# SvenGronauer/distributedTensorFlow

Measured on AMD Instinct MI355X. Metric: images/sec (whole node) ResNet-50 synthetic ImageNet at 1/2/4/8 MI355X, higher is better.
Workload: dtype bf16; 1 GPU; model=resnet50, global_batch=1984, per_gpu_batch=1984, image_size=224, parallelism=dp1, impl=dtf, optimizer=momentum0.9+wd1e-4, lr 0.1*B/256 warmup500+cosine, backend=auto, native_ext=distributedtensorflow_amd/_lib/_dtf_hip.cpython-310-x86_64-linux-gnu.so

## Files before the change

csrc/kernels/batchnorm.hip:

```cpp
#include <stdexcept>

#include "launch.h"

namespace {

constexpr int kThreads = 256;

static int g_bn_stats_blocks = 1024;

inline int stats_grid(long M, int C, int* rows_per_block) {
  const int tpr = C / 8;
  const int rpi = kThreads / tpr;
  long target_blocks = g_bn_stats_blocks;
  long rpb = (M + target_blocks - 1) / target_blocks;
  rpb = ((rpb + rpi - 1) / rpi) * rpi;
  if (rpb < rpi) rpb = rpi;
  *rows_per_block = (int)rpb;
  return (int)((M + rpb - 1) / rpb);
}

constexpr int kUnroll = 4;

DTF_DEV void relu_mask8(float* g, const float* xv, uint32_t mbyte, uint4 yraw, int kind,
                        const float* ksc, const float* ksh) {
  if (kind == 1) {
#pragma unroll
    for (int i = 0; i < 8; ++i) g[i] = (mbyte >> i) & 1u ? g[i] : 0.f;
  } else if (kind == 2) {
#pragma unroll
    for (int i = 0; i < 8; ++i) g[i] = __builtin_fmaf(xv[i], ksc[i], ksh[i]) > 0.f ? g[i] : 0.f;
  } else if (kind == 3) {
    float yv[8];
    unpack8(yraw, yv);
#pragma unroll
    for (int i = 0; i < 8; ++i) g[i] = yv[i] > 0.f ? g[i] : 0.f;
  }
}

DTF_DEV void load8cg(const float* __restrict__ p, int cg, float* v) {
  const float4 a = reinterpret_cast<const float4*>(p)[cg * 2];
  const float4 b = reinterpret_cast<const float4*>(p)[cg * 2 + 1];
  v[0] = a.x; v[1] = a.y; v[2] = a.z; v[3] = a.w; v[4] = b.x; v[5] = b.y; v[6] = b.z; v[7] = b.w;
}

typedef uint32_t u32x4_nt __attribute__((ext_vector_type(4)));
// ... 617 lines not shown
```

csrc/kernels/bindings.cpp:

```cpp
#include <hip/hip_runtime.h>
#include <pybind11/pybind11.h>
#include <pybind11/stl.h>

#include <algorithm>
#include <stdexcept>
#include <string>
#include <vector>

#include "launch.h"

namespace py = pybind11;

namespace dlp {
struct Device { int32_t device_type; int32_t device_id; };
struct DataType { uint8_t code; uint8_t bits; uint16_t lanes; };
struct Tensor { void* data; Device device; int32_t ndim; DataType dtype; int64_t* shape;
                int64_t* strides; uint64_t byte_offset; };
struct Managed { Tensor t; void* ctx; void (*deleter)(Managed*); };
constexpr int32_t kROCM = 10;
struct Ctx { int64_t shape[1]; int64_t strides[1]; uintptr_t ptr; int device; bool opened; };
void deleter(Managed* m) {
  auto* c = static_cast<Ctx*>(m->ctx);
  if (c->opened) dtf_ipc_close(c->ptr, c->device);
  else dtf_ipc_free(c->ptr, c->device);
// ... 446 lines not shown
             eeta, eps, gscale, nesterov, P<float>(partial), P<int>(nonfinite), S(st));
    check_launch("lars");
  });
  m.def("sumsq", [](uintptr_t x, long n, uintptr_t out, uintptr_t st) {
    dtf_sumsq(P<const float>(x), n, P<float>(out), S(st));
    check_launch("sumsq");
  });
  m.def("cast_f32_bf16", [](uintptr_t x, uintptr_t y, long n, uintptr_t st) {
    dtf_cast_f32_bf16(P<const float>(x), P<bf16_t>(y), n, S(st));
    check_launch("cast_f32_bf16");
  });
  m.def("conv_igemm", [](uintptr_t x, uintptr_t w, uintptr_t y, std::vector<int> geom,
                         std::vector<int> dh, std::vector<int> dw, int bk, uintptr_t st,
                         uintptr_t stats, std::vector<uintptr_t> bnb, uintptr_t acc_src,
                         uintptr_t acc_mask, uintptr_t bias, int relu, uintptr_t bnl_sc,
                         uintptr_t bnl_sh, uintptr_t bnl_y) {
    ConvGeom g = conv_geom("conv_igemm", geom);
    g.acc_src = P<const bf16_t>(acc_src);
    g.acc_mask = P<const uint8_t>(acc_mask);
    g.bias = P<const float>(bias);
    g.relu = relu;
    if (g.acc == 2 && (!g.acc_src || !g.acc_mask))
      throw std::runtime_error("conv_igemm: acc 2 needs acc_src and acc_mask");
    g.lsc = P<const float>(bnl_sc);
    g.lsh = P<const float>(bnl_sh);
    g.ly = P<bf16_t>(bnl_y);
    const BnBwdEpi e = bnb_epi("conv_igemm", bnb, 9);
    dtf_conv_igemm(P<const bf16_t>(x), P<const bf16_t>(w), P<bf16_t>(y), g,
                   make_taps<TapTable>(dh, dw), bk, P<float>(stats), e, S(st));
    check_launch("conv_igemm");
  }, py::arg("x"), py::arg("w"), py::arg("y"), py::arg("geom"), py::arg("dh"), py::arg("dw"),
     py::arg("bk"), py::arg("stream"), py::arg("stats") = 0,
     py::arg("bnb") = std::vector<uintptr_t>{}, py::arg("acc_src") = 0, py::arg("acc_mask") = 0,
     py::arg("bias") = 0, py::arg("relu") = 0, py::arg("bnl_sc") = 0, py::arg("bnl_sh") = 0,
     py::arg("bnl_y") = 0);
  m.def("conv_igemm_grouped", [](uintptr_t x, uintptr_t y, std::vector<int> geom,
                                 std::vector<uintptr_t> wts, std::vector<int> oh0,
                                 std::vector<int> ow0, std::vector<int> kpad,
                                 std::vector<std::vector<int>> dh, std::vector<std::vector<int>> dw,
                                 uintptr_t st, std::vector<uintptr_t> bnb, std::vector<int> row0) {
    if (geom.size() != 17) throw std::runtime_error("conv_igemm_grouped: geom needs 17 ints");
    const size_t n = wts.size();
    if (oh0.size() != n || ow0.size() != n || kpad.size() != n || dh.size() != n ||
        dw.size() != n || (!bnb.empty() && row0.size() != n))
      throw std::runtime_error("conv_igemm_grouped: per-class lists differ in length");
    const ConvGeom g = conv_geom("conv_igemm_grouped", geom);
    const BnBwdEpi e = bnb_epi("conv_igemm_grouped", bnb, 8);
    std::vector<const bf16_t*> w(n);
    for (size_t i = 0; i < n; ++i) w[i] = P<const bf16_t>(wts[i]);
    const bool ok = dtf_conv_igemm_grouped(P<const bf16_t>(x), P<bf16_t>(y), g, (int)n, w.data(),
                                           oh0.data(), ow0.data(), kpad.data(), dh, dw, e,
                                           row0.empty() ? nullptr : row0.data(), S(st));
    if (ok) check_launch("conv_igemm_grouped");
    return ok;
  });
  m.def("gemm_conv_part_images", &dtf_gemm_conv_part_images);
  m.def("gemm_set_pp2_strided", &dtf_gemm_set_pp2_strided);
  m.def("conv_bnl_ok", [](std::vector<int> geom, std::vector<int> dh, std::vector<int> dw) {
    const ConvGeom g = conv_geom("conv_bnl_ok", geom);
    return dtf_conv_bnl_ok(g, make_taps<TapTable>(dh, dw));
  });
  m.def("bn_bwd_finalize_g", [](uintptr_t part, int G, long M, int C, uintptr_t gamma,
                                uintptr_t mean, uintptr_t invstd, uintptr_t dg, uintptr_t db,
                                uintptr_t a, uintptr_t b, uintptr_t c, int accumulate,
                                uintptr_t st) {
    dtf_bn_bwd_finalize_g(P<const float>(part), G, M, C, P<const float>(gamma),
                          P<const float>(mean), P<const float>(invstd), P<float>(dg), P<float>(db),
                          P<float>(a), P<float>(b), P<float>(c), accumulate, S(st));
    check_launch("bn_bwd_finalize_g");
  });
  m.def("conv_wgrad", [](uintptr_t x, uintptr_t dy, uintptr_t dw_out, uintptr_t ws,
                         std::vector<int> geom, std::vector<int> dh, std::vector<int> dw,
                         int splits, uintptr_t st, int tr_mode, int accumulate) {
    if (geom.size() != 10) throw std::runtime_error("conv_wgrad: geom needs 10 ints");
    WgradGeom g{geom[0], geom[1], geom[2], geom[3], geom[4], geom[5], geom[6], geom[7], geom[8],
// ... 235 lines not shown
```

csrc/kernels/common.h:

```cpp
#pragma once
#include <hip/hip_runtime.h>
#include <stdint.h>

#define DTF_DEV __device__ __forceinline__

typedef uint16_t bf16_t;
typedef __attribute__((ext_vector_type(8))) short bf16x8_t;
typedef __attribute__((ext_vector_type(4))) short bf16x4_t;
typedef __attribute__((ext_vector_type(4))) float f32x4_t;
typedef __attribute__((ext_vector_type(16))) float f32x16_t;

DTF_DEV float bf2f(bf16_t v) { return __builtin_bit_cast(float, ((uint32_t)v) << 16); }
DTF_DEV bf16_t f2bf(float f) { return __builtin_bit_cast(bf16_t, (__bf16)f); }

DTF_DEV void unpack8(const uint4& v, float* f) {
  const uint32_t w[4] = {v.x, v.y, v.z, v.w};
#pragma unroll
  for (int i = 0; i < 4; ++i) {
    f[2 * i] = __builtin_bit_cast(float, w[i] << 16);
    f[2 * i + 1] = __builtin_bit_cast(float, w[i] & 0xffff0000u);
  }
}
DTF_DEV uint32_t pack2(float a, float b) {
  return (uint32_t)f2bf(a) | ((uint32_t)f2bf(b) << 16);
// ... 65 lines not shown
#define DTF_WAIT_VM(n) asm volatile("s_waitcnt vmcnt(" #n ")" ::: "memory")
template <int N>
DTF_DEV void wait_vm() {
  static_assert(N >= 0 && N < 64, "vmcnt range");
  asm volatile("s_waitcnt vmcnt(%0)" ::"n"(N) : "memory");
}
DTF_DEV void raw_barrier() {
  asm volatile("" ::: "memory");
  __builtin_amdgcn_s_barrier();
  asm volatile("" ::: "memory");
}

DTF_DEV float bn_bwd_dx(float a, float dz, float b, float x, float c) {
  return __builtin_fmaf(a, dz, b * x) + c;
}

DTF_DEV void pool3s2_gather(const uint4 (&dyr)[4], const uint2 (&amr)[4], int a, int b, int P,
                            int Q, float (&g)[4][8]) {
#pragma unroll
  for (int k = 0; k < 4; ++k)
#pragma unroll
    for (int e = 0; e < 8; ++e) g[k][e] = 0.f;
#pragma unroll
  for (int da = 0; da < 2; ++da) {
    if (a + da >= P) continue;
#pragma unroll
    for (int db = 0; db < 2; ++db) {
      if (b + db >= Q) continue;
      float gv[8];
      unpack8(dyr[da * 2 + db], gv);
// ... 49 lines not shown
```

csrc/kernels/conv.hip:

```cpp
#include <algorithm>
#include <stdexcept>
#include <string>
#include <vector>

#include "launch.h"

DTF_DEV uint4 acc_add8(const ConvGeom& g, const bf16_t* Y, long off, uint4 v) {
  float a[8], b[8];
  unpack8(v, a);
  if (g.acc == 2) {
    unpack8(*reinterpret_cast<const uint4*>(g.acc_src + off), b);
    const uint32_t m = g.acc_mask[off >> 3];
#pragma unroll
    for (int e = 0; e < 8; ++e) b[e] = (m >> e) & 1u ? b[e] : 0.f;
  } else {
    unpack8(*reinterpret_cast<const uint4*>(Y + off), b);
  }
#pragma unroll
  for (int e = 0; e < 8; ++e) a[e] += b[e];
  return pack8(a);
}

static int g_small_k = 31;

// ... 666 lines not shown
  static constexpr int LDC = NT + 8;
  static constexpr size_t LDS = (size_t)(PIXAL * C + 2 * WST) * 2;
  static constexpr size_t lds(int st, int nstg = 2) {
    return (size_t)(st * PIXAL * C + nstg * WST) * 2;
  }
  static constexpr size_t LDS_FREG = (size_t)PIXAL * C * 2;
  static_assert(M % (16 * WMW) == 0 && NT % (16 * WNW) == 0, "halo tiling");
  static_assert((size_t)M * LDC * 2 + (size_t)2 * NT * (kThreads / NT) * 4 <= (size_t)PIXAL * C * 2,
                "halo epilogue must fit in the patch region");
};

template <int C>
DTF_DEV int halo_swz(int u) { return C == 64 ? (((u >> 1) & 3) << 1) : ((u & 7) << 1); }

template <int C, int W, int WMW, int NT, int ST = 1, bool FREG = false, bool BNB = false,
          int NSTG = 2, bool BNL = false, int BNLP = 0>
__global__ void __launch_bounds__(kThreads * ST, ST == 1 ? 2 : 1)
conv3x3_halo_kernel(const bf16_t* __restrict__ X, const bf16_t* __restrict__ Wt,
                    bf16_t* __restrict__ Y, const ConvGeom g, const TapTable taps,
                    float* __restrict__ stats, const BnBwdEpi bnb) {
  using H = HaloCfg<C, W, WMW, NT>;
  static_assert(!BNL || (!FREG && ST == 1 && !BNB), "BN on load: the forward ring kernel");
  extern __shared__ __attribute__((aligned(16))) bf16_t lds[];
  const int tid = threadIdx.x & (kThreads - 1), lane = tid & 63;
  const int wall = __builtin_amdgcn_readfirstlane((int)threadIdx.x >> 6);
  const int sid = wall >> 2, wave = wall & 3;
  bf16_t* const patch = lds + sid * (H::PIXAL * C);
  bf16_t* const wst = lds + ST * (H::PIXAL * C);
  float* const bnl_prm = reinterpret_cast<float*>(wst + NSTG * H::WST);
  if constexpr (BNL) {
    for (int t = tid; t < C / 4; t += kThreads) {
      const int ch = t >> 1, half = t & 1;
      reinterpret_cast<float4*>(bnl_prm)[ch * 4 + half] =
          *reinterpret_cast<const float4*>(g.lsc + 4 * t);
      reinterpret_cast<float4*>(bnl_prm)[ch * 4 + 2 + half] =
          *reinterpret_cast<const float4*>(g.lsh + 4 * t);
    }
  }
  const int wm = wave / H::WNW, wn = wave % H::WNW;
  const int tiles_h = g.H / kHaloTH;
  const int tm = blockIdx.x * ST + sid;
  const bool live = tm < g.N * tiles_h;
  const int n = live ? tm / tiles_h : 0, h0 = live ? (tm % tiles_h) * kHaloTH : 0;
  const int n0 = blockIdx.y * NT;
  const i32x4_t rx = rsrc_quad(X + (long)n * g.H * g.W * g.C, (uint32_t)g.H * g.W * g.C * 2u);
  const i32x4_t rw = rsrc_quad(Wt, (uint32_t)g.Kout * g.Kpad * 2u);
  const uint32_t lds_patch = lds_addr(patch), lds_w = lds_addr(wst);

  {
    constexpr int CPP = H::ROWB / 16;
    const int lp = lane / CPP, slot = lane % CPP;
    for (int q = wave; q < H::PIXAL / H::PPI; q += 4) {
      const int pix = q * H::PPI + lp;
// ... 3 lines not shown
      const bool ok = live && pix < H::PIX && (unsigned)h < (unsigned)g.H &&
                      (unsigned)w < (unsigned)g.W;
      const uint32_t off = ok ? (uint32_t)(((h * g.W + w) * C + chunk * 8) * 2) : kOOB;
      dma16(rx, lds_patch + (uint32_t)q * 1024u, off);
    }
  }
  constexpr int OCPR = NT / 8;
  constexpr int OROWS = kThreads / OCPR;
  constexpr int NR = H::M / OROWS;
  static_assert(H::M % OROWS == 0, "halo epilogue rows");
  const long ybase = ((long)n * g.H + h0) * g.W;
  const int oc = tid % OCPR;
  const bool col_ok = n0 + oc * 8 < g.Kout;
  uint4 xpre[BNB ? NR : 1];
  uint32_t mpre[BNB ? NR : 1];
  if constexpr (BNB) {
#pragma unroll
    for (int k = 0; k < NR; ++k) {
      const long off = (ybase + tid / OCPR + k * OROWS) * g.Kout + n0 + oc * 8;
      const bool ok = live && col_ok;
      xpre[k] = ok ? *reinterpret_cast<const uint4*>(bnb.x + off) : make_uint4(0, 0, 0, 0);
      mpre[k] = (ok && bnb.mkind == 1) ? (uint32_t)bnb.mask[off >> 3] : 0u;
    }
  }
  const int lp8 = lane >> 3, slot8 = lane & 7;
  auto issue_w = [&](int step, int stage) {
    const int t = step / H::KS, s = step - t * H::KS;
#pragma unroll
    for (int i = 0; i < NT / (32 * ST); ++i) {
      const int q = wall + 4 * ST * i;
      const int row = q * 8 + lp8;
      const int chunk = slot8 ^ ((row >> 1) & 7);
      const int kr = n0 + row;
      const uint32_t off = (t < taps.n && kr < g.Kout)
                               ? (uint32_t)((kr * g.Kpad + t * C + s * 64 + chunk * 8) * 2) : kOOB;
      dma16(rw, lds_w + (uint32_t)(stage * H::WST) * 2u + (uint32_t)q * 1024u, off);
    }
// ... 64 lines not shown
        for (int i = 0; i < H::MF; ++i) {
          const int p = pbase[i] + dpix;
          const bf16x8_t af = *reinterpret_cast<const bf16x8_t*>(
              patch + p * C + ((pch ^ halo_swz<C>(ubase[i] + dupix)) << 3));
#pragma unroll
          for (int j = 0; j < H::NF; ++j)
            acc[i][j] = __builtin_amdgcn_mfma_f32_16x16x32_bf16(af, cur[ks][j], acc[i][j], 0, 0, 0);
        }
      }
      __builtin_amdgcn_sched_barrier(0);
      if (step + D < NSTEP) ldB(step + D, cur);
      __builtin_amdgcn_sched_barrier(0);
    }
  } else {
  const int nsteps = taps.n * H::KS;
  for (int step = 0; step < nsteps; ++step) {
    if constexpr (kYoung == 0) DTF_WAIT_VM(0);
    else if constexpr (kYoung == 1) DTF_WAIT_VM(1);
    else if constexpr (kYoung == 2) DTF_WAIT_VM(2);
    else if constexpr (kYoung == 3) DTF_WAIT_VM(3);
    else if constexpr (kYoung == 4) DTF_WAIT_VM(4);
    else if constexpr (kYoung == 6) DTF_WAIT_VM(6);
    else DTF_WAIT_VM(8);
    __syncthreads();
    if constexpr (BNL) {
      if (step == 0) {
        constexpr int CPP = H::ROWB / 16;
        constexpr int ITEMS = (H::PIX * CPP + kThreads - 1) / kThreads;
#pragma unroll
        for (int k = 0; k < ITEMS; ++k) {
          const int idx = tid + k * kThreads;
          const int pix = idx / CPP, slot = idx - pix * CPP;
          const int pr = pix / H::PW, pc = pix - pr * H::PW;
          const int h = h0 - 1 + pr, w = pc - 1;
          if (idx >= H::PIX * CPP || (unsigned)h >= (unsigned)g.H || (unsigned)w >= (unsigned)g.W)
            continue;
          const int lch = slot ^ halo_swz<C>(pr * W + pc);
          uint4* pp = reinterpret_cast<uint4*>(patch + pix * C + slot * 8);
// ... 307 lines not shown
                            : conv3x3_halo_kernel<C, W, WMW, NT, 1, false, false, 2, true>;
#else
    auto kern = conv3x3_halo_kernel<C, W, WMW, NT, 1, false, false, 2, true>;
#endif
    const size_t lds = Hc::lds(1) + (size_t)2 * C * sizeof(float);
    static bool attr[2] = {false, false};
    if (!attr[g_bnl_probe ? 1 : 0]) {
      HIP_CHECK(hipFuncSetAttribute((const void*)kern, hipFuncAttributeMaxDynamicSharedMemorySize,
                                    (int)lds));
      attr[g_bnl_probe ? 1 : 0] = true;
    }
    hipLaunchKernelGGL(kern, dim3((unsigned)tiles, g.Kout / NT), dim3(kThreads), lds, st,
                       X, Wt, Y, g, taps, stats, bnb);
    return;
  }
  if (!freg_on && (nstg == 3 || nstg == 4)) {
    if (bnb.part) {
      constexpr size_t scratch =
          (size_t)Hc::M * Hc::LDC * 2 + (size_t)(kThreads / (NT / 8)) * 2 * NT * 4;
      const size_t base = Hc::lds(1, nstg);
      const size_t lds = base > scratch ? base : scratch;
      if (nstg == 3) launch_halo_ring<C, W, WMW, NT, 1, true, 3>(X, Wt, Y, g, taps, stats, bnb, tiles, lds, st);
      else launch_halo_ring<C, W, WMW, NT, 1, true, 4>(X, Wt, Y, g, taps, stats, bnb, tiles, lds, st);
    } else if (strips == 2) {
      if (nstg == 3) launch_halo_ring<C, W, WMW, NT, 2, false, 3>(X, Wt, Y, g, taps, stats, bnb, tiles, Hc::lds(2, 3), st);
      else launch_halo_ring<C, W, WMW, NT, 2, false, 4>(X, Wt, Y, g, taps, stats, bnb, tiles, Hc::lds(2, 4), st);
    } else {
      if (nstg == 3) launch_halo_ring<C, W, WMW, NT, 1, false, 3>(X, Wt, Y, g, taps, stats, bnb, tiles, Hc::lds(1, 3), st);
      else launch_halo_ring<C, W, WMW, NT, 1, false, 4>(X, Wt, Y, g, taps, stats, bnb, tiles, Hc::lds(1, 4), st);
    }
// ... 79 lines not shown
  if (use_conv_gemm(g, taps)) return (int)(((long)g.N * g.P * g.Q + 255) / 256);
  if (g.C % 32 == 0 && use_halo(g, taps)) return g.N * (g.H / kHaloTH);
  if (use_stem_halo(g, taps)) return g.N * (g.P / kStemTH);
  const long M = (long)g.N * g.P * g.Q;
  return dtf_conv_stats_rows(M, g.Kout, g.C, taps.n, 0);
}

static int g_conv_nt = 0;
void dtf_conv_set_nt(int v) { g_conv_nt = v; }

bool dtf_conv_bnl_ok(const ConvGeom& g, const TapTable& taps) {
  const int fam = halo_family(g, taps);
  if (!fam || (g_halo_freg & fam) || (g_halo_st & fam)) return false;
  const int nstg = (g_halo_stages >> (fam == 1 ? 0 : 4)) & 15;
  return nstg != 3 && nstg != 4;
}

void dtf_conv_igemm(const bf16_t* X, const bf16_t* Wt, bf16_t* Y, const ConvGeom& g_in,
                    const TapTable& taps, int bk, float* stats, const BnBwdEpi& bnb,
                    hipStream_t st) {
  ConvGeom g = g_in;
  g.nt = g_conv_nt;
  if (bnb.part && (stats || !bnb.x || !bnb.mean || !bnb.invstd ||
                   (bnb.mkind == 1 && !bnb.mask) || (bnb.mkind == 2 && !(bnb.fsc && bnb.fsh))))
    throw std::runtime_error("conv: bad fused BN-backward epilogue arguments");
  if (taps.n <= 0 || taps.n > DTF_MAX_TAPS) throw std::runtime_error("conv: bad tap count");
  if (g.Kout % 8) throw std::runtime_error("conv: Kout % 8 != 0");
  const double ibytes = 2.0 * g.H * g.W * g.C, wbytes = 2.0 * g.Kout * g.Kpad;
  const double m = (double)g.N * g.P * g.Q;
  const double span = (double)(255 / (g.P * g.Q) + 2);
// ... 2 lines not shown
    throw std::runtime_error("conv: image / filter too large for 32-bit buffer offsets");
  const bool narrow = g.Kout <= 64;
  const bool epi = g.bias || g.relu;
  if (epi && (bnb.part || g.acc))
    throw std::runtime_error("conv: fused bias/ReLU epilogue excludes BN / accumulate epilogues");
  if (g.ly) {
    if (!dtf_conv_bnl_ok(g, taps) || !g.lsc || !g.lsh || bnb.part || epi)
      throw std::runtime_error("conv: BN on load needs a halo-family forward conv");
    const int tiles = g.N * (g.H / kHaloTH);
    if (halo_family(g, taps) == 1)
      launch_halo<64, 56, 2, 64>(X, Wt, Y, g, taps, stats, bnb, tiles, 1, st);
    else
      launch_halo<128, 28, 1, 128>(X, Wt, Y, g, taps, stats, bnb, tiles, 1, st);
    return;
  }
  if (!bnb.part && use_stem_halo(g, taps)) {
    using Sc = StemCfg<112>;
    static bool attr = false;
    if (!attr) {
      HIP_CHECK(hipFuncSetAttribute((const void*)conv_stem_halo_kernel<112>,
                                    hipFuncAttributeMaxDynamicSharedMemorySize, (int)Sc::LDS));
      attr = true;
    }
    hipLaunchKernelGGL(conv_stem_halo_kernel<112>, dim3((unsigned)(g.N * (g.P / kStemTH))),
                       dim3(kThreads), Sc::LDS, st, X, Wt, Y, g, stats);
    return;
  }
  if (g.C % 32 != 0) {
    if (g.Kpad % 32) throw std::runtime_error("conv: Kpad % 32 != 0");
    if (g.C % 8 == 0) {
// ... 153 lines not shown
```

csrc/kernels/launch.h:

```cpp
#pragma once
#include <string>
#include <vector>

#include "common.h"

#define DTF_MAX_TAPS 64

struct TapTable {
  int n;
  int dh[DTF_MAX_TAPS];
  int dw[DTF_MAX_TAPS];
};

struct TapTableW {
  int n;
  int dh[DTF_MAX_TAPS];
  int dw[DTF_MAX_TAPS];
};

struct ConvGeom {
  int N, H, W, C;
  int P, Q;
  int sh, sw;
  int Kout;
  int Kpad;
  int Ho, Wo;
  int osh, osw, oh0, ow0;
  int acc;
  const bf16_t* acc_src;
  const uint8_t* acc_mask;
  const float* bias;
  int relu;
  int nt;
  const float* lsc;
  const float* lsh;
  bf16_t* ly;
};

struct BnBwdEpi {
  const bf16_t* x;
  const float* mean;
  const float* invstd;
  const float* fsc;
  const float* fsh;
  const uint8_t* mask;
  float* part;
  int mkind;
  int row0;
};

constexpr int kWtMaxJobs = 48;
// ... 63 lines not shown

void dtf_conv_set_small_k(int mode);
void dtf_conv_set_dma_mode(int mode);
void dtf_conv_set_halo(int on);
void dtf_conv_set_halo_strips(int v);
void dtf_conv_set_halo_freg(int v);
void dtf_conv_set_halo_stages(int v);
void dtf_conv_set_bnl_probe(int v);
void dtf_conv_set_stem_halo(int v);
void dtf_conv_set_halo_bnb(int v);
int dtf_conv_stats_rows(long M, int Kout, int C, int taps, int W);
void dtf_conv_set_gemm(int v);
int dtf_conv_tile_rows(const ConvGeom& g, const TapTable& taps, int bnb);
void dtf_conv_set_nt(int v);
bool dtf_conv_bnl_ok(const ConvGeom& g, const TapTable& taps);
void dtf_conv_igemm(const bf16_t* X, const bf16_t* Wt, bf16_t* Y, const ConvGeom& g_in,
                    const TapTable& taps, int bk, float* stats, const BnBwdEpi& bnb,
                    hipStream_t st);
bool dtf_conv_igemm_grouped(const bf16_t* X, bf16_t* Y, const ConvGeom& g0, int ncls,
                            const bf16_t* const* wts, const int* oh0, const int* ow0,
                            const int* kpad, const std::vector<std::vector<int>>& dh,
                            const std::vector<std::vector<int>>& dw, const BnBwdEpi& bnb,
                            const int* row0, hipStream_t st);
void dtf_filter_transpose(const WtJobs& jobs, hipStream_t st);

void dtf_wgrad_set_dma_mode(int mode);
void dtf_wgrad_set_pp(int v);
void dtf_wgrad_set_dense(int v);
void dtf_wgrad_set_deep(int v);
void dtf_wgrad_set_direct(int v);
// ... 241 lines not shown
```

distributedtensorflow_amd/ops/native.py:

```python
from __future__ import annotations

import os

import torch

from .records import BnDeferred as _BnDeferred
from .records import GradSlot as _GradSlot
from .records import LazyBnDx as _LazyBnDx
from .records import LazyStemDz as _LazyStemDz
from .records import MaskedGrad as _MaskedGrad
from .records import Recompute as _Recompute
from .records import end_step as end_step
from .reference import resolve_padding, space_to_depth_operands

try:
    from .._lib import _dtf_hip as _K
except ImportError as e:
    raise ImportError(
        "distributedtensorflow_amd HIP extension (_lib/_dtf_hip*.so) is not built; run "
        "`python -m distributedtensorflow_amd._build` (hipcc --offload-arch=gfx950). "
        f"Original error: {e}") from e

_BF16 = torch.bfloat16
_DENSE_IMPL = os.environ.get("DTF_DENSE", "native")
# ... 91 lines not shown
    sh, sw = _pair(stride)
    pt, pb, pl, pr = resolve_padding(padding, h, w, R, S, stride)
    P = (h + pt + pb - R) // sh + 1
    Q = (w + pl + pr - S) // sw + 1
    return n, h, w, c, P, Q, sh, sw, pt, pl


def _fwd_geom(xshape, K, taps, P, Q, sh, sw, Ho, Wo, osh=1, osw=1, oh0=0, ow0=0, accumulate=False):
    n, h, w, c = xshape
    kpad = -(-(len(taps) * c) // 32) * 32
    return [n, h, w, c, P, Q, sh, sw, K, kpad, Ho, Wo, osh, osw, oh0, ow0, int(accumulate)]


def _launch_fwd(x, wmat, K, taps, P, Q, sh, sw, out, Ho, Wo, osh=1, osw=1, oh0=0, ow0=0,
                stats=None, accumulate=False, bnb=(), acc_from=None, bias=None, relu=False,
                bnl=None):
    n, h, w, c = x.shape
    dh = [t[0] for t in taps]
    dw = [t[1] for t in taps]
    kdim = len(taps) * c
    kpad = -(-kdim // 32) * 32
    if kpad != kdim:
        padded = torch.zeros(K, kpad, device=x.device, dtype=_BF16)
        padded[:, :kdim] = wmat
        wmat = padded
    geom = [n, h, w, c, P, Q, sh, sw, K, kpad, Ho, Wo, osh, osw, oh0, ow0,
            2 if acc_from is not None else int(accumulate)]
    if acc_from is not None:
        if tuple(acc_from.dy.shape) != tuple(out.shape) or acc_from.dy.dtype != _BF16:
            raise ValueError("masked residual gradient does not match the dgrad output")
        _K.conv_igemm(x.data_ptr(), wmat.data_ptr(), out.data_ptr(), geom, dh, dw, 64, _st(),
                      _p(stats), list(bnb), acc_from.dy.data_ptr(), acc_from.mask.data_ptr())
        return
    if bnl is not None:
        _K.conv_igemm(bnl.x.data_ptr(), wmat.data_ptr(), out.data_ptr(), geom, dh, dw, 64, _st(),
                      _p(stats), list(bnb), 0, 0, 0, 0, bnl.scale.data_ptr(),
                      bnl.shift.data_ptr(), bnl.y().data_ptr())
        bnl.done = True
        return
    _K.conv_igemm(x.data_ptr(), wmat.data_ptr(), out.data_ptr(), geom, dh, dw, 64, _st(),
                  _p(stats), list(bnb), 0, 0, _p(bias), int(relu))


def _bnl_pending(x):
    rec = getattr(x, "_dtf_bnl", None)
    return rec if rec is not None and not rec.done else None


def conv2d_forward(x, w_bf16, stride, padding, stats=None, bias=None, relu=False):
    K, R, S, C = w_bf16.shape
    n, h, wd, c, P, Q, sh, sw, pt, pl = _conv_geom_fwd(x, K, R, S, stride, padding)
    assert c == C, (x.shape, w_bf16.shape)
    if bias is None and not relu and _gemm_1x1(C, K, R, S, stride, (pt, pl)) and \
            x.is_contiguous() and w_bf16.is_contiguous():
# ... 36 lines not shown
        _WT_PENDING.clear()
        _WT_CACHE.clear()
        outs = [torch.empty(w.shape[3], w.shape[1] * w.shape[2], w.shape[0], device=w.device,
                            dtype=_BF16) for w in items]
        _K.filter_transpose([w.data_ptr() for w in items], [o.data_ptr() for o in outs],
                            [w.shape[0] for w in items], [w.shape[1] * w.shape[2] for w in items],
                            [w.shape[3] for w in items], _st())
        for w, o in zip(items, outs):
            _WT_CACHE[w.data_ptr()] = o
        t = _WT_CACHE.get(key)
        if t is not None and t.shape == (wflat.shape[2], wflat.shape[1], wflat.shape[0]):
            return t
    return wflat.permute(2, 1, 0).contiguous()


def conv2d_dgrad(dy, w_bf16, x_shape, stride, padding, out=None, bnb=None, acc_from=None):
    K, R, S, C = w_bf16.shape
    n, h, wd, c = x_shape
    sh, sw = _pair(stride)
    pt, pb, pl, pr = resolve_padding(padding, h, wd, R, S, stride)
    dx = None
    wflat = w_bf16.reshape(K, R * S, C)
    if isinstance(bnb, _DualBnb) and not (_gemm_1x1(K, C, R, S, stride, (pt, pl)) and
                                          _stream_bnb_ok(K, C)):
        bnb = None
    if _gemm_1x1(K, C, R, S, stride, (pt, pl)) and (bnb is None or _stream_bnb_ok(K, C)):
        M = n * h * wd
        wt = _dgrad_filter(wflat).view(C, K)
        dyc = dy.contiguous().view(M, K)
        if bnb is not None:
            return _dgrad_1x1_bnb(dyc, wt, M, C, K, (n, h, wd, C), out, acc_from, bnb)
# ... 59 lines not shown
        mats = [class_filter(l[5]).reshape(C, -1) for l in launches]
        Pc, Qc = launches[0][2], launches[0][3]
        geom = _fwd_geom(dyc.shape, C, launches[0][4], Pc, Qc, 1, 1, h, wd, sh, sw, 0, 0, acc)
        if _K.conv_igemm_grouped(dyc.data_ptr(), dx.data_ptr(), geom,
                                 [m.data_ptr() for m in mats], [l[0] for l in launches],
                                 [l[1] for l in launches], [len(l[4]) * K for l in launches],
                                 [[t[0] for t in l[4]] for l in launches],
                                 [[t[1] for t in l[4]] for l in launches], _st(), [], []):
            return dx
    for li, (a, b, Pc, Qc, taps, idx) in enumerate(launches):
        wd_mat = class_filter(idx)
        extra = ()
        if part is not None:
            extra = base + [row0]
            row0 += rows[li]
        _launch_fwd(dyc, wd_mat.reshape(C, -1), C, taps, Pc, Qc, 1, 1, dx, h, wd, sh, sw, a, b,
                    accumulate=acc, bnb=extra, acc_from=acc_from)
    if part is not None:
        dx._dtf_bnb_part = (part, G, n * h * wd, C, tok, dx._version)
    return dx


def _stream_bnb_ok(K, C):
    return _GEMM_STREAM and K in (64, 128, 256) and C >= K and C % 64 == 0 and C <= 2048


class _DualBnb:
    __slots__ = ("x", "stats", "mask", "xp", "stats_p", "tok")

    def __init__(self, x, stats, mask, xp, stats_p, tok):
        self.x, self.stats, self.mask, self.xp, self.stats_p, self.tok = \
            x, stats, mask, xp, stats_p, tok
# ... 139 lines not shown
                  and (_FUSE_BN_BWD_S2_ALL or xb.shape[-1] < 256))
        ctx.bnb = bnb if ((_FUSE_BN_BWD or stream_bnb or halo_bnb or s2_bnb) and bnb is not None
                          and xb is x) else None
        dual = getattr(x, "_dtf_bnb_dual", None)
        if dual is not None and stream_bnb and ctx.bnb is None and xb is x:
            ctx.bnb = _DualBnb(*dual)
        if x.requires_grad and xb is x and wb.is_contiguous():
            _register_dgrad_filter(wb)
        out = conv2d_forward(xb, wb, stride, padding, stats)
        ctx.stem_slot = None
        if (_FUSE_STEM_WGRAD and not x.requires_grad and _stem_wgrad_shape(xb, wb, stride, padding)
                and _K.wgrad_stem_dz_splits(xb.shape[0]) > 0):
            ctx.stem_slot = _GradSlot()
            out._dtf_stem_slot = ctx.stem_slot
            ctx.set_materialize_grads(False)
        return out

    @staticmethod
    def backward(ctx, dy):
        xb, wb = ctx.saved_tensors
        dx = dw = None
        C = ctx.c_orig
        padded = xb.shape[-1] != C
        slot, ctx.stem_slot = ctx.stem_slot, None
        rec = None
        if slot is not None:
            rec, slot.grad = slot.grad, None
        if dy is None and rec is None:
            ctx.x_ref = ctx.bnb = ctx.share = None
            return None, None, None, None, None, None
        if rec is not None and (dy is not None or not ctx.needs_input_grad[1]):
            m = rec.materialize()
            dy = m if dy is None else dy + m
            rec = None
        if rec is not None:
            target = _direct_grad(ctx.w_param)
            K, R, S, _ = wb.shape
            n = xb.shape[0]
            splits = _K.wgrad_stem_dz_splits(n)
            dW = target if target is not None else torch.empty(K, R * S * C, device=xb.device,
                                                                dtype=torch.float32)
            ws = torch.empty(splits * K * R * S * C, device=xb.device, dtype=torch.float32)
            _K.conv_wgrad_stem_dz(xb.data_ptr(), rec.dp.data_ptr(), rec.arg.data_ptr(),
                                  rec.x.data_ptr(), rec.gb[2].data_ptr(), rec.gb[3].data_ptr(),
                                  rec.gb[4].data_ptr(), rec.fsc.data_ptr(), rec.fsh.data_ptr(),
# ... 127 lines not shown
_FUSE_BN_BWD = os.environ.get("DTF_FUSE_BN_BWD", "0") == "1"
_FUSE_BN_BWD_STREAM = os.environ.get("DTF_FUSE_BN_BWD_STREAM", "1") == "1"


_FUSE_BN_BWD_HALO = os.environ.get("DTF_FUSE_BN_BWD_HALO", "1") == "1"
_FUSE_BN_BWD_S2 = os.environ.get("DTF_FUSE_BN_BWD_S2", "1") == "1"
_DGRAD_GROUPED = os.environ.get("DTF_DGRAD_GROUPED", "1") == "1"
_FUSE_BN_BWD_S2_ALL = os.environ.get("DTF_FUSE_BN_BWD_S2_ALL", "0") == "1"


def _halo_dgrad_shape(K, C, H, W):
    return H % 4 == 0 and ((K == 64 and W == 56 and C % 64 == 0) or
                           (K == 128 and W == 28 and C % 128 == 0))


def conv2d(x, w, stride=1, padding=0, bn_stats=False, grad_share=None):
    _check_cuda_bf16(x)
    K, R, S, C = w.shape
    if K % 8 or R * S > 64:
        raise ValueError(f"native conv2d: unsupported filter {tuple(w.shape)}")
    if grad_share is not None and (x.shape[-1] % 8 or not _SHARE_INPUT_GRAD):
        grad_share = None
    if not bn_stats:
        return _Conv2d.apply(x, w, stride, padding, None, grad_share)
    n, h, wd, c, P, Q, sh, sw, pt, pl = _conv_geom_fwd(x, K, R, S, stride, padding)
    M = n * P * Q
    taps = [(r - pt, s - pl) for r in range(R) for s in range(S)]
    cp = -(-c // 8) * 8
    if _gemm_1x1(cp, K, R, S, stride, (pt, pl)):
        G = _K.gemm_tile_rows(M)
# ... 165 lines not shown
                         invstd.data_ptr(), M, C, int(relu), part.data_ptr(), st,
                         sc_ptr, sh_ptr, _p(mask))
    gb, direct = _bn_bwd_finalize(ctx, part, G, M, C, g32, stats)
    dx = torch.empty_like(x) if getattr(ctx, "in_slot", None) is None else None
    lazy = (ctx.has_res and ctx.res_ref is not None and _LAZY_RESIDUAL_GRAD
            and mask is not None)
    res_slot = getattr(ctx, "res_slot", None)
    lazy_slot = (ctx.has_res and not lazy and res_slot is not None and _LAZY_RESIDUAL_GRAD
                 and mask is not None)
    dres = torch.empty_like(x) if ctx.has_res and not (lazy or lazy_slot) else None
    in_slot = getattr(ctx, "in_slot", None)
    ctx.in_slot = None
    if in_slot is not None and dres is None and mask is not None and relu:
        in_slot.grad = _LazyBnDx(dy, x, mask, gb)
        dx = None
    else:
        if dx is None:
            dx = torch.empty_like(x)
        _materialized(x)
        _K.bn_bwd_apply(dy.data_ptr(), 0, x.data_ptr(), gb[2].data_ptr(),
                        gb[3].data_ptr(), gb[4].data_ptr(), dx.data_ptr(), _p(dres), M, C,
                        int(relu), st, sc_ptr, sh_ptr, _p(mask))
    if lazy:
        ctx.res_ref._dtf_pending_grad = _MaskedGrad(dy, mask)
    elif lazy_slot:
        res_slot.grad = _MaskedGrad(dy, mask)
        ctx.res_slot = None
    elif dres is not None and ctx.res_ref is not None:
        ctx.res_ref._dtf_pending_grad = dres
        dres = None
# ... 37 lines not shown
                           stats[2].data_ptr(), stats[3].data_ptr(), y.data_ptr(),
                           part.data_ptr(), _st(), int(lazy))
        out._dtf_bn_part = (part, G, M, K)
        if lazy:
            out._dtf_recompute = _Recompute(y, wb, out)
        if wb.is_contiguous():
            _register_dgrad_filter(wb)
        ctx.lz_slot = None
        if _FUSE_C1_BWD and _FUSE_C3_LAZY and _K.conv1x1_bwd_lazy_ok(M, C, K):
            ctx.lz_slot = _GradSlot()
            out._dtf_lazy_slot = ctx.lz_slot
            ctx.set_materialize_grads(False)
        ctx.save_for_backward(x, y, wb, g32, stats)
        ctx.w_param, ctx.w_dtype = w_master, w_master.dtype
        ctx.relu, ctx.has_res, ctx.res_ref, ctx.res_slot = True, False, None, None
        ctx.params = (gamma, beta)
        ctx.gdt, ctx.bdt = gamma.dtype, beta.dtype
        return out

    @staticmethod
    def backward(ctx, dout):
        x, y, wb, g32, stats = ctx.saved_tensors
        lz, ctx.lz_slot = ctx.lz_slot, None
        rec = lz.grad if lz is not None else None
        if lz is not None:
            lz.grad = None
        if dout is None and rec is None:
            ctx.w_param = ctx.params = None
            return (None,) * 9
        if dout is not None and rec is not None:
# ... 837 lines not shown
```

distributedtensorflow_amd/ops/records.py:

```python
from __future__ import annotations

import contextlib
import weakref

_LIVE = weakref.WeakSet()


class ReleasedRecordError(RuntimeError):
    """A deferred-work record was used after the step that created it ended."""


class _Record:
    __slots__ = ("released", "__weakref__")

    def __init__(self):
        self.released = False
        _LIVE.add(self)

    def _check(self):
        if self.released:
            raise ReleasedRecordError(
                f"{type(self).__name__} used after its training step ended (records are "
                "released by ops.end_step(), called after every backward)")

# ... 99 lines not shown
        self.dp, self.arg, self.x, self.gb = dp, arg, x, gb
        self.fsc, self.fsh, self.geom = fsc, fsh, geom

    def materialize(self):
        self._check()
        n = _native()
        N, H, W, C, P, Q = self.geom
        dx = self.x.new_empty(self.x.shape)
        n._K.pool_bn_bwd_apply(self.dp.data_ptr(), self.arg.data_ptr(), self.x.data_ptr(),
                               self.gb[2].data_ptr(), self.gb[3].data_ptr(),
                               self.gb[4].data_ptr(), self.fsc.data_ptr(), self.fsh.data_ptr(),
                               dx.data_ptr(), N, H, W, C, P, Q, n._st())
        return dx


class GradSlot(_Record):
    __slots__ = ("grad",)

    def __init__(self):
        super().__init__()
        self.grad = None

    def release(self):
        g = self.grad
        super().release()
        if isinstance(g, _Record):
            g.release()


def live_count():
# ... 7 lines not shown
    _LIVE.clear()
    return len(recs)


@contextlib.contextmanager
def isolated():
    global _LIVE
    outer, _LIVE = _LIVE, weakref.WeakSet()
    try:
        yield
    finally:
        end_step()
        _LIVE = outer


__all__ = ["BnDeferred", "Recompute", "MaskedGrad", "LazyBnDx", "LazyStemDz", "GradSlot",
           "ReleasedRecordError", "live_count", "end_step", "isolated"]
```

Baseline: 17370 images/sec.

## Fuse BN backward apply into the 3x3 halo dgrad conv load

Adds a BNZ variant of the 3x3 halo conv kernel. At patch-load time it applies the BN-backward data-gradient transform (ReLU gate recomputed from x, scale and shift, then the a*dz + b*x + c affine) to the incoming gradient tile, and writes dz out as a side product for the weight gradient. The BN backward apply is deferred on the Python side through a new LazyBnDz record, so the following conv dgrad can consume it without a separate elementwise kernel and an extra read of the full gradient tensor. It costs extra register pressure (the per-channel parameters and prefetched x), a full vmem wait before the first step, and more complex lazy-grad plumbing with fallback paths.

New measurement: 17300 images/sec. Within noise of the previous version (-0.4%).

```diff
diff --git a/csrc/kernels/batchnorm.hip b/csrc/kernels/batchnorm.hip
--- a/csrc/kernels/batchnorm.hip
+++ b/csrc/kernels/batchnorm.hip
@@ -28,7 +28,7 @@
     for (int i = 0; i < 8; ++i) g[i] = (mbyte >> i) & 1u ? g[i] : 0.f;
   } else if (kind == 2) {
 #pragma unroll
-    for (int i = 0; i < 8; ++i) g[i] = __builtin_fmaf(xv[i], ksc[i], ksh[i]) > 0.f ? g[i] : 0.f;
+    for (int i = 0; i < 8; ++i) g[i] = bn_bwd_gate(g[i], xv[i], ksc[i], ksh[i]);
   } else if (kind == 3) {
     float yv[8];
     unpack8(yraw, yv);
diff --git a/csrc/kernels/bindings.cpp b/csrc/kernels/bindings.cpp
--- a/csrc/kernels/bindings.cpp
+++ b/csrc/kernels/bindings.cpp
@@ -484,8 +484,21 @@
                          std::vector<int> dh, std::vector<int> dw, int bk, uintptr_t st,
                          uintptr_t stats, std::vector<uintptr_t> bnb, uintptr_t acc_src,
                          uintptr_t acc_mask, uintptr_t bias, int relu, uintptr_t bnl_sc,
-                         uintptr_t bnl_sh, uintptr_t bnl_y) {
+                         uintptr_t bnl_sh, uintptr_t bnl_y, std::vector<uintptr_t> bnz) {
     ConvGeom g = conv_geom("conv_igemm", geom);
+    if (!bnz.empty()) {
+      if (bnz.size() != 7 || bnl_y)
+        throw std::runtime_error("conv_igemm: bnz needs [x, scale, shift, A, B, C, dz] and no bnl");
+      for (uintptr_t p : bnz)
+        if (!p) throw std::runtime_error("conv_igemm: null bnz operand");
+      g.zx = P<const bf16_t>(bnz[0]);
+      g.zsc = P<const float>(bnz[1]);
+      g.zsh = P<const float>(bnz[2]);
+      g.za = P<const float>(bnz[3]);
+      g.zb = P<const float>(bnz[4]);
+      g.zc = P<const float>(bnz[5]);
+      g.dz = P<bf16_t>(bnz[6]);
+    }
     g.acc_src = P<const bf16_t>(acc_src);
     g.acc_mask = P<const uint8_t>(acc_mask);
     g.bias = P<const float>(bias);
@@ -503,7 +516,7 @@
      py::arg("bk"), py::arg("stream"), py::arg("stats") = 0,
      py::arg("bnb") = std::vector<uintptr_t>{}, py::arg("acc_src") = 0, py::arg("acc_mask") = 0,
      py::arg("bias") = 0, py::arg("relu") = 0, py::arg("bnl_sc") = 0, py::arg("bnl_sh") = 0,
-     py::arg("bnl_y") = 0);
+     py::arg("bnl_y") = 0, py::arg("bnz") = std::vector<uintptr_t>{});
   m.def("conv_igemm_grouped", [](uintptr_t x, uintptr_t y, std::vector<int> geom,
                                  std::vector<uintptr_t> wts, std::vector<int> oh0,
                                  std::vector<int> ow0, std::vector<int> kpad,
@@ -529,6 +542,10 @@
   m.def("conv_bnl_ok", [](std::vector<int> geom, std::vector<int> dh, std::vector<int> dw) {
     const ConvGeom g = conv_geom("conv_bnl_ok", geom);
     return dtf_conv_bnl_ok(g, make_taps<TapTable>(dh, dw));
+  });
+  m.def("conv_bnz_ok", [](std::vector<int> geom, std::vector<int> dh, std::vector<int> dw) {
+    const ConvGeom g = conv_geom("conv_bnz_ok", geom);
+    return dtf_conv_bnz_ok(g, make_taps<TapTable>(dh, dw));
   });
   m.def("bn_bwd_finalize_g", [](uintptr_t part, int G, long M, int C, uintptr_t gamma,
                                 uintptr_t mean, uintptr_t invstd, uintptr_t dg, uintptr_t db,
diff --git a/csrc/kernels/common.h b/csrc/kernels/common.h
--- a/csrc/kernels/common.h
+++ b/csrc/kernels/common.h
@@ -103,6 +103,9 @@
 DTF_DEV float bn_bwd_dx(float a, float dz, float b, float x, float c) {
   return __builtin_fmaf(a, dz, b * x) + c;
 }
+DTF_DEV float bn_bwd_gate(float g, float x, float sc, float sh) {
+  return __builtin_fmaf(x, sc, sh) > 0.f ? g : 0.f;
+}
 
 DTF_DEV void pool3s2_gather(const uint4 (&dyr)[4], const uint2 (&amr)[4], int a, int b, int P,
                             int Q, float (&g)[4][8]) {
diff --git a/csrc/kernels/conv.hip b/csrc/kernels/conv.hip
--- a/csrc/kernels/conv.hip
+++ b/csrc/kernels/conv.hip
@@ -704,13 +704,15 @@
 DTF_DEV int halo_swz(int u) { return C == 64 ? (((u >> 1) & 3) << 1) : ((u & 7) << 1); }
 
 template <int C, int W, int WMW, int NT, int ST = 1, bool FREG = false, bool BNB = false,
-          int NSTG = 2, bool BNL = false, int BNLP = 0>
+          int NSTG = 2, bool BNL = false, int BNLP = 0, bool BNZ = false>
 __global__ void __launch_bounds__(kThreads * ST, ST == 1 ? 2 : 1)
 conv3x3_halo_kernel(const bf16_t* __restrict__ X, const bf16_t* __restrict__ Wt,
                     bf16_t* __restrict__ Y, const ConvGeom g, const TapTable taps,
                     float* __restrict__ stats, const BnBwdEpi bnb) {
   using H = HaloCfg<C, W, WMW, NT>;
   static_assert(!BNL || (!FREG && ST == 1 && !BNB), "BN on load: the forward ring kernel");
+  static_assert(!BNZ || (!FREG && ST == 1 && NSTG == 2 && BNB && !BNL),
+                "BN backward on load: the default ring kernel with the BN-sum epilogue");
   extern __shared__ __attribute__((aligned(16))) bf16_t lds[];
   const int tid = threadIdx.x & (kThreads - 1), lane = tid & 63;
   const int wall = __builtin_amdgcn_readfirstlane((int)threadIdx.x >> 6);
@@ -727,6 +729,20 @@
           *reinterpret_cast<const float4*>(g.lsh + 4 * t);
     }
   }
+  constexpr int ZCPP = H::ROWB / 16;
+  static_assert(kThreads % ZCPP == 0, "BNZ: one chunk per thread");
+  const int zch = tid % ZCPP;
+  float zprm[BNZ ? 5 : 1][8];
+  if constexpr (BNZ) {
+    const float* const src[5] = {g.zsc, g.zsh, g.za, g.zb, g.zc};
+#pragma unroll
+    for (int p = 0; p < 5; ++p) {
+      const float4 a = *reinterpret_cast<const float4*>(src[p] + zch * 8);
+      const float4 b = *reinterpret_cast<const float4*>(src[p] + zch * 8 + 4);
+      zprm[p][0] = a.x; zprm[p][1] = a.y; zprm[p][2] = a.z; zprm[p][3] = a.w;
+      zprm[p][4] = b.x; zprm[p][5] = b.y; zprm[p][6] = b.z; zprm[p][7] = b.w;
+    }
+  }
   const int wm = wave / H::WNW, wn = wave % H::WNW;
   const int tiles_h = g.H / kHaloTH;
   const int tm = blockIdx.x * ST + sid;
@@ -760,13 +776,29 @@
   const bool col_ok = n0 + oc * 8 < g.Kout;
   uint4 xpre[BNB ? NR : 1];
   uint32_t mpre[BNB ? NR : 1];
-  if constexpr (BNB) {
+  auto load_xpre = [&]() {
 #pragma unroll
     for (int k = 0; k < NR; ++k) {
       const long off = (ybase + tid / OCPR + k * OROWS) * g.Kout + n0 + oc * 8;
       const bool ok = live && col_ok;
       xpre[k] = ok ? *reinterpret_cast<const uint4*>(bnb.x + off) : make_uint4(0, 0, 0, 0);
       mpre[k] = (ok && bnb.mkind == 1) ? (uint32_t)bnb.mask[off >> 3] : 0u;
+    }
+  };
+  if constexpr (BNB && !BNZ) load_xpre();
+  constexpr int ZITEMS = (H::PIX * ZCPP + kThreads - 1) / kThreads;
+  uint4 zx[BNZ ? ZITEMS : 1];
+  if constexpr (BNZ) {
+#pragma unroll
+    for (int k = 0; k < ZITEMS; ++k) {
+      const int pix = (tid + k * kThreads) / ZCPP;
+      const int pr = pix / H::PW, pc = pix - pr * H::PW;
+      const int h = h0 - 1 + pr, w = pc - 1;
+      const bool ok = live && pix < H::PIX && (unsigned)h < (unsigned)g.H &&
+                      (unsigned)w < (unsigned)g.W;
+      zx[k] = ok ? *reinterpret_cast<const uint4*>(
+                       g.zx + (((long)n * g.H + h) * g.W + w) * C + zch * 8)
+                 : make_uint4(0, 0, 0, 0);
     }
   }
   const int lp8 = lane >> 3, slot8 = lane & 7;
@@ -861,14 +893,43 @@
     }
   } else {
   const int nsteps = taps.n * H::KS;
+  if constexpr (BNZ) {
+    DTF_WAIT_VM(0);
+    __syncthreads();
+    __builtin_amdgcn_sched_barrier(0);
+#pragma unroll
+    for (int k = 0; k < ZITEMS; ++k) {
+      const int pix = (tid + k * kThreads) / ZCPP;
+      const int pr = pix / H::PW, pc = pix - pr * H::PW;
+      const int h = h0 - 1 + pr, w = pc - 1;
+      if (!live || pix >= H::PIX || (unsigned)h >= (unsigned)g.H || (unsigned)w >= (unsigned)g.W)
+        continue;
+      const int slot = zch ^ halo_swz<C>(pr * W + pc);
+      uint4* pp = reinterpret_cast<uint4*>(patch + pix * C + slot * 8);
+      float gv[8], xv[8], o[8];
+      unpack8(*pp, gv);
+      unpack8(zx[k], xv);
+#pragma unroll
+      for (int e = 0; e < 8; ++e)
+        o[e] = bn_bwd_dx(zprm[2][e], bn_bwd_gate(gv[e], xv[e], zprm[0][e], zprm[1][e]),
+                         zprm[3][e], xv[e], zprm[4][e]);
+      const uint4 pk = pack8(o);
+      *pp = pk;
+      if (pr >= 1 && pr <= kHaloTH)
+        *reinterpret_cast<uint4*>(g.dz + (((long)n * g.H + h) * g.W + w) * C + zch * 8) = pk;
+    }
+    load_xpre();
+  }
   for (int step = 0; step < nsteps; ++step) {
-    if constexpr (kYoung == 0) DTF_WAIT_VM(0);
-    else if constexpr (kYoung == 1) DTF_WAIT_VM(1);
-    else if constexpr (kYoung == 2) DTF_WAIT_VM(2);
-    else if constexpr (kYoung == 3) DTF_WAIT_VM(3);
-    else if constexpr (kYoung == 4) DTF_WAIT_VM(4);
-    else if constexpr (kYoung == 6) DTF_WAIT_VM(6);
-    else DTF_WAIT_VM(8);
+    if (!BNZ || step != 0) {
+      if constexpr (kYoung == 0) DTF_WAIT_VM(0);
+      else if constexpr (kYoung == 1) DTF_WAIT_VM(1);
+      else if constexpr (kYoung == 2) DTF_WAIT_VM(2);
+      else if constexpr (kYoung == 3) DTF_WAIT_VM(3);
+      else if constexpr (kYoung == 4) DTF_WAIT_VM(4);
+      else if constexpr (kYoung == 6) DTF_WAIT_VM(6);
+      else DTF_WAIT_VM(8);
+    }
     __syncthreads();
     if constexpr (BNL) {
       if (step == 0) {
@@ -1206,6 +1267,26 @@
                        X, Wt, Y, g, taps, stats, bnb);
     return;
   }
+  if (g.dz) {
+    if (!bnb.part || freg_on || nstg == 3 || nstg == 4 || strips != 1)
+      throw std::runtime_error("halo conv: BN backward on load needs the default ring kernel "
+                               "with the BN-sum epilogue");
+    auto kern = conv3x3_halo_kernel<C, W, WMW, NT, 1, false, true, 2, false, 0, true>;
+    constexpr size_t scratch =
+        (size_t)Hc::M * Hc::LDC * 2 + (size_t)(kThreads / (NT / 8)) * 2 * NT * 4;
+    static_assert(scratch <= Hc::lds(1), "halo BNZ: BN-sum scratch within patch + ring");
+    constexpr size_t lds = Hc::lds(1);
+    static_assert(2 * lds <= 160 * 1024, "halo BNZ: two blocks per CU");
+    static bool attr = false;
+    if (!attr) {
+      HIP_CHECK(hipFuncSetAttribute((const void*)kern, hipFuncAttributeMaxDynamicSharedMemorySize,
+                                    (int)lds));
+      attr = true;
+    }
+    hipLaunchKernelGGL(kern, dim3((unsigned)tiles, g.Kout / NT), dim3(kThreads), lds, st,
+                       X, Wt, Y, g, taps, stats, bnb);
+    return;
+  }
   if (!freg_on && (nstg == 3 || nstg == 4)) {
     if (bnb.part) {
       constexpr size_t scratch =
@@ -1315,6 +1396,11 @@
   if (!fam || (g_halo_freg & fam) || (g_halo_st & fam)) return false;
   const int nstg = (g_halo_stages >> (fam == 1 ? 0 : 4)) & 15;
   return nstg != 3 && nstg != 4;
+}
+
+bool dtf_conv_bnz_ok(const ConvGeom& g, const TapTable& taps) {
+  return dtf_conv_bnl_ok(g, taps) && g_halo_bnb && g.C % 32 == 0 && !g.bias && !g.relu &&
+         g.Kout == (halo_family(g, taps) == 1 ? 64 : 128);
 }
 
 void dtf_conv_igemm(const bf16_t* X, const bf16_t* Wt, bf16_t* Y, const ConvGeom& g_in,
@@ -1347,6 +1433,18 @@
       launch_halo<128, 28, 1, 128>(X, Wt, Y, g, taps, stats, bnb, tiles, 1, st);
     return;
   }
+  if (g.dz) {
+    if (!dtf_conv_bnz_ok(g, taps) || !g.zx || !g.zsc || !g.zsh || !g.za || !g.zb || !g.zc ||
+        !bnb.part || stats || epi)
+      throw std::runtime_error("conv: BN backward on load needs a halo-family data gradient "
+                               "with the BN-sum epilogue");
+    const int tiles = g.N * (g.H / kHaloTH);
+    if (halo_family(g, taps) == 1)
+      launch_halo<64, 56, 2, 64>(X, Wt, Y, g, taps, stats, bnb, tiles, 1, st);
+    else
+      launch_halo<128, 28, 1, 128>(X, Wt, Y, g, taps, stats, bnb, tiles, 1, st);
+    return;
+  }
   if (!bnb.part && use_stem_halo(g, taps)) {
     using Sc = StemCfg<112>;
     static bool attr = false;
diff --git a/csrc/kernels/launch.h b/csrc/kernels/launch.h
--- a/csrc/kernels/launch.h
+++ b/csrc/kernels/launch.h
@@ -35,6 +35,13 @@
   const float* lsc;
   const float* lsh;
   bf16_t* ly;
+  const bf16_t* zx;
+  const float* zsc;
+  const float* zsh;
+  const float* za;
+  const float* zb;
+  const float* zc;
+  bf16_t* dz;
 };
 
 struct BnBwdEpi {
@@ -128,6 +135,7 @@
 int dtf_conv_tile_rows(const ConvGeom& g, const TapTable& taps, int bnb);
 void dtf_conv_set_nt(int v);
 bool dtf_conv_bnl_ok(const ConvGeom& g, const TapTable& taps);
+bool dtf_conv_bnz_ok(const ConvGeom& g, const TapTable& taps);
 void dtf_conv_igemm(const bf16_t* X, const bf16_t* Wt, bf16_t* Y, const ConvGeom& g_in,
                     const TapTable& taps, int bk, float* stats, const BnBwdEpi& bnb,
                     hipStream_t st);
diff --git a/distributedtensorflow_amd/ops/native.py b/distributedtensorflow_amd/ops/native.py
--- a/distributedtensorflow_amd/ops/native.py
+++ b/distributedtensorflow_amd/ops/native.py
@@ -7,6 +7,7 @@
 from .records import BnDeferred as _BnDeferred
 from .records import GradSlot as _GradSlot
 from .records import LazyBnDx as _LazyBnDx
+from .records import LazyBnDz as _LazyBnDz
 from .records import LazyStemDz as _LazyStemDz
 from .records import MaskedGrad as _MaskedGrad
 from .records import Recompute as _Recompute
@@ -129,7 +130,7 @@
 
 def _launch_fwd(x, wmat, K, taps, P, Q, sh, sw, out, Ho, Wo, osh=1, osw=1, oh0=0, ow0=0,
                 stats=None, accumulate=False, bnb=(), acc_from=None, bias=None, relu=False,
-                bnl=None):
+                bnl=None, bnz=None):
     n, h, w, c = x.shape
     dh = [t[0] for t in taps]
     dw = [t[1] for t in taps]
@@ -153,6 +154,14 @@
                       bnl.shift.data_ptr(), bnl.y().data_ptr())
         bnl.done = True
         return
+    if bnz is not None:
+        _K.conv_igemm(x.data_ptr(), wmat.data_ptr(), out.data_ptr(), geom, dh, dw, 64, _st(),
+                      _p(stats), list(bnb),
+                      bnz=[bnz.x.data_ptr(), bnz.fsc.data_ptr(), bnz.fsh.data_ptr(),
+                           bnz.gb[2].data_ptr(), bnz.gb[3].data_ptr(), bnz.gb[4].data_ptr(),
+                           bnz.dz.data_ptr()])
+        bnz.done = True
+        return
     _K.conv_igemm(x.data_ptr(), wmat.data_ptr(), out.data_ptr(), geom, dh, dw, 64, _st(),
                   _p(stats), list(bnb), 0, 0, _p(bias), int(relu))
 
@@ -219,7 +228,8 @@
     return wflat.permute(2, 1, 0).contiguous()
 
 
-def conv2d_dgrad(dy, w_bf16, x_shape, stride, padding, out=None, bnb=None, acc_from=None):
+def conv2d_dgrad(dy, w_bf16, x_shape, stride, padding, out=None, bnb=None, acc_from=None,
+                 bnz=None):
     K, R, S, C = w_bf16.shape
     n, h, wd, c = x_shape
     sh, sw = _pair(stride)
@@ -309,8 +319,11 @@
         if part is not None:
             extra = base + [row0]
             row0 += rows[li]
+        if bnz is not None and (part is None or acc or len(launches) != 1 or dyc is not bnz.dy):
+            raise RuntimeError("conv2d_dgrad: BN backward on load needs one stride-1 launch "
+                               "with the BN-sum epilogue and nothing to accumulate")
         _launch_fwd(dyc, wd_mat.reshape(C, -1), C, taps, Pc, Qc, 1, 1, dx, h, wd, sh, sw, a, b,
-                    accumulate=acc, bnb=extra, acc_from=acc_from)
+                    accumulate=acc, bnb=extra, acc_from=acc_from, bnz=bnz)
     if part is not None:
         dx._dtf_bnb_part = (part, G, n * h * wd, C, tok, dx._version)
     return dx
@@ -480,6 +493,12 @@
             ctx.stem_slot = _GradSlot()
             out._dtf_stem_slot = ctx.stem_slot
             ctx.set_materialize_grads(False)
+        ctx.dz_slot = None
+        if (_FUSE_BN2_DGRAD_LOAD and halo_bnb and ctx.bnb is not None and share is None
+                and x.requires_grad and w_master.requires_grad and _halo_dgrad_bnz_ok(out, xb)):
+            ctx.dz_slot = _GradSlot()
+            out._dtf_dz_slot = ctx.dz_slot
+            ctx.set_materialize_grads(False)
         return out
 
     @staticmethod
@@ -492,9 +511,32 @@
         rec = None
         if slot is not None:
             rec, slot.grad = slot.grad, None
-        if dy is None and rec is None:
+        zslot, ctx.dz_slot = ctx.dz_slot, None
+        zrec = None
+        if zslot is not None:
+            zrec, zslot.grad = zslot.grad, None
+        if zrec is not None and not (
+                _FUSE_BN2_DGRAD_LOAD and dy is None and ctx.needs_input_grad[0]
+                and ctx.needs_input_grad[1] and ctx.bnb is not None and ctx.share is None
+                and not padded and getattr(ctx.x_ref, "_dtf_pending_grad", None) is None):
+            m = zrec.materialize()
+            dy = m if dy is None else dy + m
+            zrec = None
+        if dy is None and rec is None and zrec is None:
             ctx.x_ref = ctx.bnb = ctx.share = None
             return None, None, None, None, None, None
+        if zrec is not None:
+            dx = conv2d_dgrad(zrec.dy, wb, xb.shape, ctx.stride, ctx.padding, bnb=ctx.bnb,
+                              bnz=zrec)
+            dz = zrec.dz
+            target = _direct_grad(ctx.w_param)
+            if target is not None:
+                conv2d_wgrad(xb, dz, wb.shape, ctx.stride, ctx.padding, out=target)
+                _grad_ready(ctx.w_param)
+            else:
+                dw = conv2d_wgrad(xb, dz, wb.shape, ctx.stride, ctx.padding).to(ctx.w_dtype)
+            ctx.x_ref = ctx.bnb = ctx.share = None
+            return dx, dw, None, None, None, None
         if rec is not None and (dy is not None or not ctx.needs_input_grad[1]):
             m = rec.materialize()
             dy = m if dy is None else dy + m
@@ -652,6 +694,16 @@
                            (K == 128 and W == 28 and C % 128 == 0))
 
 
+_FUSE_BN2_DGRAD_LOAD = True
+
+
+def _halo_dgrad_bnz_ok(out, xb):
+    n, h, wd, K = out.shape
+    taps = [(1 - r, 1 - s) for r in range(3) for s in range(3)]
+    return _K.conv_bnz_ok(_fwd_geom((n, h, wd, K), xb.shape[-1], taps, h, wd, 1, 1, h, wd),
+                          [t[0] for t in taps], [t[1] for t in taps])
+
+
 def conv2d(x, w, stride=1, padding=0, bn_stats=False, grad_share=None):
     _check_cuda_bf16(x)
     K, R, S, C = w.shape
@@ -847,6 +899,9 @@
     if in_slot is not None and dres is None and mask is not None and relu:
         in_slot.grad = _LazyBnDx(dy, x, mask, gb)
         dx = None
+    elif in_slot is not None and mask is None and relu and not ctx.has_res:
+        in_slot.grad = _LazyBnDz(dy, x.detach(), gb, stats[2], stats[3], torch.empty_like(x))
+        dx = None
     else:
         if dx is None:
             dx = torch.empty_like(x)
@@ -914,6 +969,7 @@
         ctx.save_for_backward(x, y, wb, g32, stats)
         ctx.w_param, ctx.w_dtype = w_master, w_master.dtype
         ctx.relu, ctx.has_res, ctx.res_ref, ctx.res_slot = True, False, None, None
+        ctx.in_slot = getattr(x, "_dtf_dz_slot", None)
         ctx.params = (gamma, beta)
         ctx.gdt, ctx.bdt = gamma.dtype, beta.dtype
         return out
diff --git a/distributedtensorflow_amd/ops/records.py b/distributedtensorflow_amd/ops/records.py
--- a/distributedtensorflow_amd/ops/records.py
+++ b/distributedtensorflow_amd/ops/records.py
@@ -137,6 +137,31 @@
         return dx
 
 
+class LazyBnDz(_Record):
+    __slots__ = ("dy", "x", "gb", "fsc", "fsh", "dz", "done")
+
+    def __init__(self, dy, x, gb, fsc, fsh, dz):
+        super().__init__()
+        self.dy, self.x, self.gb, self.fsc, self.fsh, self.dz = dy, x, gb, fsc, fsh, dz
+        self.done = False
+
+    def release(self):
+        super().release()
+        self.done = True
+
+    def materialize(self):
+        self._check()
+        if not self.done:
+            n = _native()
+            C = self.x.shape[-1]
+            M = self.x.numel() // C
+            n._K.bn_bwd_apply(self.dy.data_ptr(), 0, self.x.data_ptr(), self.gb[2].data_ptr(),
+                              self.gb[3].data_ptr(), self.gb[4].data_ptr(), self.dz.data_ptr(),
+                              0, M, C, 1, n._st(), self.fsc.data_ptr(), self.fsh.data_ptr(), 0)
+            self.done = True
+        return self.dz
+
+
 class GradSlot(_Record):
     __slots__ = ("grad",)
 
@@ -174,5 +199,6 @@
         _LIVE = outer
 
 
-__all__ = ["BnDeferred", "Recompute", "MaskedGrad", "LazyBnDx", "LazyStemDz", "GradSlot",
+__all__ = ["BnDeferred", "Recompute", "MaskedGrad", "LazyBnDx", "LazyStemDz", "LazyBnDz",
+           "GradSlot",
            "ReleasedRecordError", "live_count", "end_step", "isolated"]
```
